# pswpswpsw/nif

Hardware: AMD Instinct MI355X
Metric: train-step points/sec (1D-wave, batch=1M per GPU) (higher is better)
Workload: dtype f32

## Files before the change

nif_amd/csrc/k_pnet_bf16.h:

```cpp
#pragma once
#include "nif_internal.h"

typedef __bf16 pbf16x8 __attribute__((ext_vector_type(8)));
#define PBF_FWD_U4 (3 * 2 * 64)
#define PBF_BWD_U4 (2 * 2 * 64)

__device__ __forceinline__ int pbf_feat(int m, int hf, int t) { return 16 * m + 8 * (t >> 2) + 4 * hf + (t & 3); }

__device__ __forceinline__ void pbf_build(pbf16x8* fwd, pbf16x8* bwd, const float* __restrict__ theta, long w_off, int nst,
                                          int tid, int nthreads) {
  __bf16* f16 = reinterpret_cast<__bf16*>(fwd);
  __bf16* b16 = reinterpret_cast<__bf16*>(bwd);
  for (int e = tid; e < 2 * 64 * 8; e += nthreads) {
    const int t = e & 7, lane = (e >> 3) & 63, m = e >> 9;
    const int row = lane & 31, kf = pbf_feat(m, lane >> 5, t);
    {
      const float w = (kf < nst && row < nst) ? theta[w_off + (long)kf * nst + row] : 0.f;
      const __bf16 w0 = (__bf16)w;
      const float r1 = w - (float)w0;
      const __bf16 w1 = (__bf16)r1;
      f16[((0 * 2 + m) * 64 + lane) * 8 + t] = w0;
      f16[((1 * 2 + m) * 64 + lane) * 8 + t] = w1;
      f16[((2 * 2 + m) * 64 + lane) * 8 + t] = (__bf16)(r1 - (float)w1);
    }
    if (bwd) {
      const float w = (kf < nst && row < nst) ? theta[w_off + (long)row * nst + kf] : 0.f;
      const __bf16 w0 = (__bf16)w;
      b16[((0 * 2 + m) * 64 + lane) * 8 + t] = w0;
      b16[((1 * 2 + m) * 64 + lane) * 8 + t] = (__bf16)(w - (float)w0);
    }
  }
}

__device__ __forceinline__ void pbf_dense_fwd(const pbf16x8* fwd, const f32x16& h, f32x16& T, int lane) {
  pbf16x8 x0[2], x1[2], x2[2];
#pragma unroll
  for (int m = 0; m < 2; ++m)
#pragma unroll
    for (int t = 0; t < 8; ++t) {
      const float x = h[8 * m + t];
      const __bf16 a = (__bf16)x;
      const float r1 = x - (float)a;
      const __bf16 b = (__bf16)r1;
      x0[m][t] = a; x1[m][t] = b; x2[m][t] = (__bf16)(r1 - (float)b);
    }
  f32x16 acc;
#pragma unroll
  for (int e = 0; e < 16; ++e) acc[e] = 0.f;
  const pbf16x8 w0a = fwd[(0 * 2 + 0) * 64 + lane], w0b = fwd[(0 * 2 + 1) * 64 + lane];
  const pbf16x8 w1a = fwd[(1 * 2 + 0) * 64 + lane], w1b = fwd[(1 * 2 + 1) * 64 + lane];
  const pbf16x8 w2a = fwd[(2 * 2 + 0) * 64 + lane], w2b = fwd[(2 * 2 + 1) * 64 + lane];
  acc = __builtin_amdgcn_mfma_f32_32x32x16_bf16(w1a, x1[0], acc, 0, 0, 0);
  acc = __builtin_amdgcn_mfma_f32_32x32x16_bf16(w1b, x1[1], acc, 0, 0, 0);
  acc = __builtin_amdgcn_mfma_f32_32x32x16_bf16(w2a, x0[0], acc, 0, 0, 0);
  acc = __builtin_amdgcn_mfma_f32_32x32x16_bf16(w2b, x0[1], acc, 0, 0, 0);
  acc = __builtin_amdgcn_mfma_f32_32x32x16_bf16(w0a, x2[0], acc, 0, 0, 0);
  acc = __builtin_amdgcn_mfma_f32_32x32x16_bf16(w0b, x2[1], acc, 0, 0, 0);
  acc = __builtin_amdgcn_mfma_f32_32x32x16_bf16(w1a, x0[0], acc, 0, 0, 0);
  acc = __builtin_amdgcn_mfma_f32_32x32x16_bf16(w1b, x0[1], acc, 0, 0, 0);
  acc = __builtin_amdgcn_mfma_f32_32x32x16_bf16(w0a, x1[0], acc, 0, 0, 0);
  acc = __builtin_amdgcn_mfma_f32_32x32x16_bf16(w0b, x1[1], acc, 0, 0, 0);
  acc = __builtin_amdgcn_mfma_f32_32x32x16_bf16(w0a, x0[0], acc, 0, 0, 0);
  acc = __builtin_amdgcn_mfma_f32_32x32x16_bf16(w0b, x0[1], acc, 0, 0, 0);
  T = acc;
}

__device__ __forceinline__ void pbf_dense_bwd(const pbf16x8* bwd, const f32x16& ga, f32x16& U, int lane) {
  pbf16x8 x0[2], x1[2];
#pragma unroll
  for (int m = 0; m < 2; ++m)
#pragma unroll
    for (int t = 0; t < 8; ++t) {
      const float x = ga[8 * m + t];
      const __bf16 a = (__bf16)x;
      x0[m][t] = a; x1[m][t] = (__bf16)(x - (float)a);
    }
  f32x16 acc;
#pragma unroll
  for (int e = 0; e < 16; ++e) acc[e] = 0.f;
  const pbf16x8 w0a = bwd[(0 * 2 + 0) * 64 + lane], w0b = bwd[(0 * 2 + 1) * 64 + lane];
  const pbf16x8 w1a = bwd[(1 * 2 + 0) * 64 + lane], w1b = bwd[(1 * 2 + 1) * 64 + lane];
  acc = __builtin_amdgcn_mfma_f32_32x32x16_bf16(w1a, x0[0], acc, 0, 0, 0);
  acc = __builtin_amdgcn_mfma_f32_32x32x16_bf16(w1b, x0[1], acc, 0, 0, 0);
  acc = __builtin_amdgcn_mfma_f32_32x32x16_bf16(w0a, x1[0], acc, 0, 0, 0);
  acc = __builtin_amdgcn_mfma_f32_32x32x16_bf16(w0b, x1[1], acc, 0, 0, 0);
  acc = __builtin_amdgcn_mfma_f32_32x32x16_bf16(w0a, x0[0], acc, 0, 0, 0);
  acc = __builtin_amdgcn_mfma_f32_32x32x16_bf16(w0b, x0[1], acc, 0, 0, 0);
  U = acc;
}

template <int NB>
__device__ __forceinline__ void pbfn_build_fwd(pbf16x8* fwd, const float* __restrict__ theta, long w_off, int nst, int tid, int nthreads) {
  __bf16* f16 = reinterpret_cast<__bf16*>(fwd);
  for (int e = tid; e < NB * NB * 1024; e += nthreads) {
    const int t = e & 7, lane = (e >> 3) & 63, m = (e >> 9) & 1, blk = e >> 10;
    const int ob = blk / NB, ib = blk - ob * NB;
    const int row = 32 * ob + (lane & 31), kf = 32 * ib + pbf_feat(m, lane >> 5, t);
    const float w = (kf < nst && row < nst) ? theta[w_off + (long)kf * nst + row] : 0.f;
    const __bf16 w0 = (__bf16)w;
    const float r1 = w - (float)w0;
    const __bf16 w1 = (__bf16)r1;
    __bf16* q = f16 + (long)blk * PBF_FWD_U4 * 8;
    q[((0 * 2 + m) * 64 + lane) * 8 + t] = w0;
    q[((1 * 2 + m) * 64 + lane) * 8 + t] = w1;
    q[((2 * 2 + m) * 64 + lane) * 8 + t] = (__bf16)(r1 - (float)w1);
  }
}
template <int NB>
__device__ __forceinline__ void pbfn_dense_fwd(const pbf16x8* fwd, const f32x16 (&h)[NB], f32x16 (&T)[NB], int lane) {
  pbf16x8 x0[NB][2], x1[NB][2], x2[NB][2];
#pragma unroll
  for (int ib = 0; ib < NB; ++ib)
#pragma unroll
    for (int m = 0; m < 2; ++m)
#pragma unroll
      for (int t = 0; t < 8; ++t) {
        const float x = h[ib][8 * m + t];
        const __bf16 a = (__bf16)x;
        const float r1 = x - (float)a;
        const __bf16 b = (__bf16)r1;
        x0[ib][m][t] = a; x1[ib][m][t] = b; x2[ib][m][t] = (__bf16)(r1 - (float)b);
      }
#pragma unroll
  for (int ob = 0; ob < NB; ++ob) {
    f32x16 acc;
#pragma unroll
    for (int e = 0; e < 16; ++e) acc[e] = 0.f;
#pragma unroll
    for (int ib = 0; ib < NB; ++ib) {
      const pbf16x8* q = fwd + (long)(ob * NB + ib) * PBF_FWD_U4;
      const pbf16x8 w0a = q[(0 * 2 + 0) * 64 + lane], w0b = q[(0 * 2 + 1) * 64 + lane];
      const pbf16x8 w1a = q[(1 * 2 + 0) * 64 + lane], w1b = q[(1 * 2 + 1) * 64 + lane];
      const pbf16x8 w2a = q[(2 * 2 + 0) * 64 + lane], w2b = q[(2 * 2 + 1) * 64 + lane];
      acc = __builtin_amdgcn_mfma_f32_32x32x16_bf16(w1a, x1[ib][0], acc, 0, 0, 0);
      acc = __builtin_amdgcn_mfma_f32_32x32x16_bf16(w1b, x1[ib][1], acc, 0, 0, 0);
      acc = __builtin_amdgcn_mfma_f32_32x32x16_bf16(w2a, x0[ib][0], acc, 0, 0, 0);
      acc = __builtin_amdgcn_mfma_f32_32x32x16_bf16(w2b, x0[ib][1], acc, 0, 0, 0);
      acc = __builtin_amdgcn_mfma_f32_32x32x16_bf16(w0a, x2[ib][0], acc, 0, 0, 0);
      acc = __builtin_amdgcn_mfma_f32_32x32x16_bf16(w0b, x2[ib][1], acc, 0, 0, 0);
      acc = __builtin_amdgcn_mfma_f32_32x32x16_bf16(w1a, x0[ib][0], acc, 0, 0, 0);
      acc = __builtin_amdgcn_mfma_f32_32x32x16_bf16(w1b, x0[ib][1], acc, 0, 0, 0);
      acc = __builtin_amdgcn_mfma_f32_32x32x16_bf16(w0a, x1[ib][0], acc, 0, 0, 0);
      acc = __builtin_amdgcn_mfma_f32_32x32x16_bf16(w0b, x1[ib][1], acc, 0, 0, 0);
      acc = __builtin_amdgcn_mfma_f32_32x32x16_bf16(w0a, x0[ib][0], acc, 0, 0, 0);
      acc = __builtin_amdgcn_mfma_f32_32x32x16_bf16(w0b, x0[ib][1], acc, 0, 0, 0);
    }
    T[ob] = acc;
  }
}
```

nif_amd/csrc/k_pnetbw.hip:

```cpp
#include "nif_internal.h"
#include "k_pnet_bf16.h"

struct PbwArgs {
  PNetArgs p;
  float* partial; long pstride;
  const float* touch; long touch_floats;
};

__device__ __forceinline__ f32x4 lds4(const float* q) { return *reinterpret_cast<const f32x4*>(q); }

__device__ __forceinline__ int pswz(int f, int p) { return f * 32 + ((((p >> 2) ^ (f & 7))) << 2) + (p & 3); }
__device__ __forceinline__ int pswz4(int f, int c) { return f * 32 + ((c ^ (f & 7)) << 2); }
__device__ __forceinline__ void tile_store(float* __restrict__ t, const f32x16& h, int p, int hf) {
#pragma unroll
  for (int v = 0; v < 16; ++v) t[pswz(fmap(v, hf), p)] = h[v];
}

typedef __bf16 pbw_bf16x8 __attribute__((ext_vector_type(8)));
__device__ __forceinline__ void grad_mfma(const float* IN, const float* DA, f32x16& C, int i, int hf, int in_rows = 32) {
  f32x4 a[4], b[4];
#pragma unroll
  for (int q = 0; q < 4; ++q) {
    a[q] = lds4(IN + pswz4(i < in_rows ? i : 0, 4 * hf + q));
    if (i >= in_rows) { a[q][0] = 0.f; a[q][1] = 0.f; a[q][2] = 0.f; a[q][3] = 0.f; }
    b[q] = lds4(DA + pswz4(i, 4 * hf + q));
  }
#pragma unroll
  for (int hh = 0; hh < 2; ++hh) {
    pbw_bf16x8 ah, al, bh, bl;
#pragma unroll
    for (int e = 0; e < 8; ++e) {
      const float x = a[2 * hh + (e >> 2)][e & 3], y = b[2 * hh + (e >> 2)][e & 3];
      const __bf16 x0 = (__bf16)x, y0 = (__bf16)y;
      ah[e] = x0; al[e] = (__bf16)(x - (float)x0);
      bh[e] = y0; bl[e] = (__bf16)(y - (float)y0);
    }
    C = __builtin_amdgcn_mfma_f32_32x32x16_bf16(ah, bl, C, 0, 0, 0);
    C = __builtin_amdgcn_mfma_f32_32x32x16_bf16(al, bh, C, 0, 0, 0);
    C = __builtin_amdgcn_mfma_f32_32x32x16_bf16(ah, bh, C, 0, 0, 0);
  }
}
__device__ __forceinline__ float col_sum(const float* DA, int i, int hf) {
  float s = 0.f;
#pragma unroll
  for (int q = 0; q < 4; ++q) { const f32x4 b = lds4(DA + pswz4(i, 4 * hf + q)); s += (b[0] + b[1]) + (b[2] + b[3]); }
  return s;
}

#ifndef NIF_PBW_DZR
#define NIF_PBW_DZR 8
#endif
#ifndef NIF_PBW_WAVES
#define NIF_PBW_WAVES 8
#endif
template <int NM, bool RES, int ACT, bool SMALL>
__global__ __launch_bounds__(64 * NIF_PBW_WAVES) void k_pnet_bwg(PbwArgs G) {
  const PNetArgs& A = G.p;
  extern __shared__ __attribute__((aligned(16))) float lds[];
  constexpr int WV = NIF_PBW_WAVES;
  __shared__ float red[(WV - 1) * 64];
  const int lane = threadIdx.x & 63, wid = threadIdx.x >> 6;
  const int p = lane & 31, hf = lane >> 5, i = p;
  const long ntiles = (A.B + 31) / 32;
  constexpr int WLDS = (NM + 2) * 1024 + 256;
  float* hs = lds + (long)wid * WLDS;
  float* gaT = hs + (NM + 1) * 1024;
  float* xT = gaT + 1024;

  f32x16 C[NM], C1, Cb, CB1;
  float gbh[NM], gb0 = 0.f, gbb = 0.f;
#pragma unroll
  for (int e = 0; e < 16; ++e) { C1[e] = 0.f; Cb[e] = 0.f; CB1[e] = 0.f; }
#pragma unroll
  for (int m = 0; m < NM; ++m) {
    gbh[m] = 0.f;
#pragma unroll
    for (int e = 0; e < 16; ++e) C[m][e] = 0.f;
  }
  for (int q = lane; q < 256; q += 64) xT[q] = 0.f;
  const PSmall S = psmall_stage<1>(A, lds + (long)WV * WLDS, threadIdx.x, 64 * WV);
  f32x4* wpl = reinterpret_cast<f32x4*>(lds + (long)WV * WLDS + ((psmall_floats(A, 1) + 3) & ~3));
  pbf16x8* bpl = reinterpret_cast<pbf16x8*>(wpl);
#pragma unroll
  for (int m = 0; m < NM; ++m) {
    const long w_off = RES ? (m == 0 ? A.hid_w[0] : A.hid_w2[0]) : A.hid_w[m];
    pbf_build(bpl + m * (PBF_FWD_U4 + PBF_BWD_U4), bpl + m * (PBF_FWD_U4 + PBF_BWD_U4) + PBF_FWD_U4, A.theta, w_off, A.nst,
              threadIdx.x, 64 * WV);
  }
  auto dense_f = [&](int m, const f32x16 (&x)[1], f32x16 (&y)[1]) { pbf_dense_fwd(bpl + m * (PBF_FWD_U4 + PBF_BWD_U4), x[0], y[0], lane); };
  auto dense_b = [&](int m, const f32x16 (&x)[1], f32x16 (&y)[1]) { pbf_dense_bwd(bpl + m * (PBF_FWD_U4 + PBF_BWD_U4) + PBF_FWD_U4, x[0], y[0], lane); };
  __syncthreads();

  for (long tile = (long)blockIdx.x * WV + wid; tile < ntiles; tile += (long)gridDim.x * WV) {
    const long pt = tile * 32 + p;
    const long ptc = pt < A.B ? pt : A.B - 1;
    const float* prow = A.xin + ptc * A.ncol + A.col0;
    float dzr[NIF_PBW_DZR];
    if (!SMALL) {
      const float* dzg = A.DZ + tile * A.r * 32;
      const int nd = A.r * 32;
#pragma unroll
      for (int q = 0; q < NIF_PBW_DZR; ++q) { const int e = lane + 64 * q; dzr[q] = e < nd ? dzg[e] : 0.f; }
    }
    f32x16 h[1], T[1], d[NM + 1][1];
    {
      f32x16 acc;
#pragma unroll
      for (int v = 0; v < 16; ++v) acc[v] = 0.f;
      for (int dd = 0; dd < A.pi; ++dd) acc += prow[dd] * psmall_get(S.fw + dd * 32, 0, hf);
      h[0] = A.omega * acc + psmall_get(S.fb, 0, hf);
    }
    act_tile_sel<1, ACT>(A.act, h, h, d[0], A.nst, hf);
    float* park = hs + NM * 1024;
    if (SMALL) {
#pragma unroll
      for (int v = 0; v < 16; ++v) park[v * 64 + lane] = d[0][0][v];
    }
    if (!SMALL && hf == 0) {
      for (int dd = 0; dd < A.pi; ++dd) xT[pswz(dd, p)] = prow[dd];
      xT[pswz(A.pi, p)] = 1.0f;
    }
    if (!RES) {
#pragma unroll
      for (int m = 0; m < NM; ++m) {
        tile_store(hs + m * 1024, h[0], p, hf);
        dense_f(m, h, T);
        T[0] = A.omega * T[0] + psmall_get(S.hb + m * 32, 0, hf);
        act_tile_sel<1, ACT>(A.act, T, T, d[m + 1], A.nst, hf);
        h[0] = A.siren ? T[0] : h[0] + T[0];
      }
    } else {
      f32x16 t[1];
      tile_store(hs, h[0], p, hf);
      dense_f(0, h, T);
      T[0] = A.omega * T[0] + psmall_get(S.hb, 0, hf);
      act_tile_sel<1, ACT>(A.act, T, t, d[1], A.nst, hf);
      tile_store(hs + 1024, t[0], p, hf);
      dense_f(1, t, T);
      {
        const f32x16 lin = A.omega * T[0] + psmall_get(S.hb2, 0, hf);
        T[0] = A.siren ? lin : h[0] + lin;
      }
      act_tile_sel<1, ACT>(A.act, T, T, d[NM], A.nst, hf);
      h[0] = A.siren ? 0.5f * (h[0] + T[0]) : T[0];
    }
    if (!SMALL) tile_store(hs + NM * 1024, h[0], p, hf);
    f32x16 gh[1], ga[1], U[1];
#pragma unroll
    for (int v = 0; v < 16; ++v) gh[0][v] = 0.f;
    if (!SMALL) {
#pragma unroll
      for (int q = 0; q < NIF_PBW_DZR; ++q) gaT[pswz(2 * q + hf, p)] = dzr[q];
#pragma unroll
      for (int q = NIF_PBW_DZR; q < 16; ++q) {
        const int e = lane + 64 * q;
        gaT[pswz(2 * q + hf, p)] = e < A.r * 32 ? A.DZ[tile * A.r * 32 + e] : 0.f;
      }
      for (int c = 0; c < A.r; ++c) gh[0] += gaT[pswz(c, p)] * psmall_get(S.bw + c * 32, 0, hf);
    } else {
      gh[0] += A.DZ[tile * 32 + p] * psmall_get(S.bw, 0, hf);
    }
    if (SMALL) {
      const float dz = A.DZ[tile * 32 + p];
      Cb += dz * h[0];
      gbb += hf == 0 ? dz : 0.f;
    } else {
      grad_mfma(hs + NM * 1024, gaT, Cb, i, hf);
      gbb += col_sum(gaT, i, hf);
    }
    float tv[4] = {0.f, 0.f, 0.f, 0.f};
    if (G.touch) {
      const float* tb = G.touch + tile * G.touch_floats + lane * 16;
#pragma unroll
      for (int q = 0; q < 4; ++q) tv[q] = tb[q * 1024 < G.touch_floats ? q * 1024 : 0];
    }
    if (!RES) {
#pragma unroll
      for (int m = NM - 1; m >= 0; --m) {
        ga[0] = gh[0] * d[m + 1][0];
        tile_store(gaT, ga[0], p, hf);
        grad_mfma(hs + m * 1024, gaT, C[m], i, hf);
        gbh[m] += col_sum(gaT, i, hf);
        dense_b(m, ga, U);
        gh[0] = A.siren ? A.omega * U[0] : gh[0] + A.omega * U[0];
      }
    } else {
      const float half = A.siren ? 0.5f : 1.0f;
      ga[0] = half * gh[0] * d[NM][0];
      tile_store(gaT, ga[0], p, hf);
      grad_mfma(hs + 1024, gaT, C[NM - 1], i, hf);
      gbh[NM - 1] += col_sum(gaT, i, hf);
      dense_b(1, ga, U);
      f32x16 skip;
      skip = A.siren ? 0.5f * gh[0] : ga[0];
      ga[0] = A.omega * U[0] * d[1][0];
      tile_store(gaT, ga[0], p, hf);
      grad_mfma(hs, gaT, C[0], i, hf);
      gbh[0] += col_sum(gaT, i, hf);
      dense_b(0, ga, U);
      gh[0] = skip + A.omega * U[0];
    }
    if (SMALL) {
#pragma unroll
      for (int v = 0; v < 16; ++v) ga[0][v] = gh[0][v] * park[v * 64 + lane];
    } else {
      ga[0] = gh[0] * d[0][0];
    }
    if (SMALL) {
      C1 += prow[0] * ga[0];
      CB1 += ga[0];
    } else {
      tile_store(gaT, ga[0], p, hf);
      grad_mfma(xT, gaT, C1, i, hf, 8);
    }
    asm volatile("" ::"v"(tv[0]), "v"(tv[1]), "v"(tv[2]), "v"(tv[3]));
  }

  float* prow_out = G.partial + (long)blockIdx.x * G.pstride;
  auto sum8 = [&](float v) -> float {
    if (wid > 0) red[(wid - 1) * 64 + lane] = v;
    __syncthreads();
    if (wid == 0) {
#pragma unroll
      for (int w = 0; w < WV - 1; ++w) v += red[w * 64 + lane];
    }
    __syncthreads();
    return v;
  };
  __syncthreads();
  auto sum16 = [&](f32x16 v) -> f32x16 {
    if (wid > 0) {
#pragma unroll
      for (int e = 0; e < 16; ++e) lds[((wid - 1) * 16 + e) * 64 + lane] = v[e];
    }
    __syncthreads();
    if (wid == 0) {
#pragma unroll
      for (int w = 0; w < WV - 1; ++w)
#pragma unroll
        for (int e = 0; e < 16; ++e) v[e] += lds[(w * 16 + e) * 64 + lane];
    }
    __syncthreads();
    return v;
  };
#pragma unroll
  for (int m = 0; m < NM; ++m) {
    const long w_off = RES ? (m == 0 ? A.hid_w[0] : A.hid_w2[0]) : A.hid_w[m];
    const long b_off = RES ? (m == 0 ? A.hid_b[0] : A.hid_b2[0]) : A.hid_b[m];
    {
      const f32x16 vs = sum16(C[m]);
#pragma unroll
      for (int e = 0; e < 16; ++e) {
        const int in = fmap(e, hf), out = i;
        if (wid == 0 && in < A.nst && out < A.nst) prow_out[w_off + (long)in * A.nst + out] = A.omega * vs[e];
      }
    }
    float vb = gbh[m];
    vb += __shfl_xor(vb, 32);
    vb = sum8(vb);
    if (wid == 0 && hf == 0 && i < A.nst) prow_out[b_off + i] = vb;
  }
  if (SMALL) {
    auto lanes32 = [&](f32x16 v) -> f32x16 {
#pragma unroll
      for (int off = 16; off > 0; off >>= 1)
#pragma unroll
        for (int e = 0; e < 16; ++e) v[e] += __shfl_xor(v[e], off);
      return v;
    };
    const f32x16 s1 = sum16(lanes32(C1)), s0 = sum16(lanes32(CB1)), sb = sum16(lanes32(Cb));
#pragma unroll
    for (int e = 0; e < 16; ++e) {
      const int f = fmap(e, hf);
      if (wid == 0 && p == 0 && f < A.nst) {
        prow_out[A.first_w + f] = A.omega * s1[e];
        prow_out[A.first_b + f] = s0[e];
        prow_out[A.bott_w + f] = sb[e];
      }
    }
    float v = gbb;
#pragma unroll
    for (int off = 32; off > 0; off >>= 1) v += __shfl_xor(v, off);
    v = sum8(v);
    if (wid == 0 && lane == 0) prow_out[A.bott_b] = v;
    return;
  }
  const f32x16 s1 = sum16(C1), sb = sum16(Cb);
#pragma unroll
  for (int e = 0; e < 16; ++e) {
    const float v1 = s1[e];
    const float vb = sb[e];
    const int row = fmap(e, hf);
    if (wid == 0) {
      if (row < A.pi && i < A.nst) prow_out[A.first_w + (long)row * A.nst + i] = A.omega * v1;
      if (row == A.pi && i < A.nst) prow_out[A.first_b + i] = v1;
      if (row < A.nst && i < A.r) prow_out[A.bott_w + (long)row * A.r + i] = vb;
    }
  }
  (void)gb0;
  {
    float v = gbb;
    v += __shfl_xor(v, 32);
    v = sum8(v);
    if (wid == 0 && hf == 0 && i < A.r) prow_out[A.bott_b + i] = v;
  }
}

bool pnet_bwg_supported(const PNetArgs& a) {
  const int nm = a.lst * (a.res ? 2 : 1);
  return a.nst <= 32 && a.pi <= 6 && a.r <= 32 && nm >= 1 && nm <= 2 && (!a.res || a.lst == 1);
}

void launch_pnet_bwg(const PNetArgs& a, float* partial, long pstride, int rows, hipStream_t st, const float* touch,
                     long touch_floats) {
  PbwArgs G; G.p = a; G.partial = partial; G.pstride = pstride; G.touch = touch; G.touch_floats = touch_floats;
  const int nm = a.lst * (a.res ? 2 : 1);
  dim3 grid(rows), block(64 * NIF_PBW_WAVES);
  const size_t shm = ((size_t)NIF_PBW_WAVES * ((nm + 2) * 1024 + 256) + (size_t)((psmall_floats(a, 1) + 3) & ~3) +
                      (size_t)nm * 2560) * sizeof(float);
#define PBW1(NM_, RES_, ACT_, SM_)                                                                                  \
  {                                                                                                                 \
    (void)hipFuncSetAttribute((const void*)k_pnet_bwg<NM_, RES_, ACT_, SM_>, hipFuncAttributeMaxDynamicSharedMemorySize, (int)shm); \
    hipLaunchKernelGGL((k_pnet_bwg<NM_, RES_, ACT_, SM_>), grid, block, shm, st, G);                                \
  }
#define PBW(NM_, RES_, ACT_)                                                                                        \
  {                                                                                                                 \
    if (a.pi == 1 && a.r == 1) PBW1(NM_, RES_, ACT_, true) else PBW1(NM_, RES_, ACT_, false)                        \
  }
#define PBWA(NM_, RES_)                                                       \
  if (a.act == ACT_SWISH) PBW(NM_, RES_, ACT_SWISH)                           \
  else if (a.act == ACT_SINE) PBW(NM_, RES_, ACT_SINE)                        \
  else PBW(NM_, RES_, -1)
  if (a.res) { PBWA(2, true) }
  else if (nm == 1) { PBWA(1, false) }
  else { PBWA(2, false) }
#undef PBWA
#undef PBW
#undef PBW1
}
```

Baseline: 942.3 million.

## Exchange bf16-split activations via LDS transpose reads for weight-gradient MFMAs

```diff
diff --git a/nif_amd/csrc/k_pnet_bf16.h b/nif_amd/csrc/k_pnet_bf16.h
--- a/nif_amd/csrc/k_pnet_bf16.h
+++ b/nif_amd/csrc/k_pnet_bf16.h
@@ -32,8 +32,7 @@
   }
 }
 
-__device__ __forceinline__ void pbf_dense_fwd(const pbf16x8* fwd, const f32x16& h, f32x16& T, int lane) {
-  pbf16x8 x0[2], x1[2], x2[2];
+__device__ __forceinline__ void pbf_split3(const f32x16& h, pbf16x8 (&x0)[2], pbf16x8 (&x1)[2], pbf16x8 (&x2)[2]) {
 #pragma unroll
   for (int m = 0; m < 2; ++m)
 #pragma unroll
@@ -44,6 +43,20 @@
       const __bf16 b = (__bf16)r1;
       x0[m][t] = a; x1[m][t] = b; x2[m][t] = (__bf16)(r1 - (float)b);
     }
+}
+__device__ __forceinline__ void pbf_split2(const f32x16& h, pbf16x8 (&x0)[2], pbf16x8 (&x1)[2]) {
+#pragma unroll
+  for (int m = 0; m < 2; ++m)
+#pragma unroll
+    for (int t = 0; t < 8; ++t) {
+      const float x = h[8 * m + t];
+      const __bf16 a = (__bf16)x;
+      x0[m][t] = a; x1[m][t] = (__bf16)(x - (float)a);
+    }
+}
+
+__device__ __forceinline__ void pbf_dense_fwd(const pbf16x8* fwd, const pbf16x8 (&x0)[2], const pbf16x8 (&x1)[2],
+                                              const pbf16x8 (&x2)[2], f32x16& T, int lane) {
   f32x16 acc;
 #pragma unroll
   for (int e = 0; e < 16; ++e) acc[e] = 0.f;
@@ -64,17 +77,13 @@
   acc = __builtin_amdgcn_mfma_f32_32x32x16_bf16(w0b, x0[1], acc, 0, 0, 0);
   T = acc;
 }
+__device__ __forceinline__ void pbf_dense_fwd(const pbf16x8* fwd, const f32x16& h, f32x16& T, int lane) {
+  pbf16x8 x0[2], x1[2], x2[2];
+  pbf_split3(h, x0, x1, x2);
+  pbf_dense_fwd(fwd, x0, x1, x2, T, lane);
+}
 
-__device__ __forceinline__ void pbf_dense_bwd(const pbf16x8* bwd, const f32x16& ga, f32x16& U, int lane) {
-  pbf16x8 x0[2], x1[2];
-#pragma unroll
-  for (int m = 0; m < 2; ++m)
-#pragma unroll
-    for (int t = 0; t < 8; ++t) {
-      const float x = ga[8 * m + t];
-      const __bf16 a = (__bf16)x;
-      x0[m][t] = a; x1[m][t] = (__bf16)(x - (float)a);
-    }
+__device__ __forceinline__ void pbf_dense_bwd(const pbf16x8* bwd, const pbf16x8 (&x0)[2], const pbf16x8 (&x1)[2], f32x16& U, int lane) {
   f32x16 acc;
 #pragma unroll
   for (int e = 0; e < 16; ++e) acc[e] = 0.f;
@@ -87,6 +96,11 @@
   acc = __builtin_amdgcn_mfma_f32_32x32x16_bf16(w0a, x0[0], acc, 0, 0, 0);
   acc = __builtin_amdgcn_mfma_f32_32x32x16_bf16(w0b, x0[1], acc, 0, 0, 0);
   U = acc;
+}
+__device__ __forceinline__ void pbf_dense_bwd(const pbf16x8* bwd, const f32x16& ga, f32x16& U, int lane) {
+  pbf16x8 x0[2], x1[2];
+  pbf_split2(ga, x0, x1);
+  pbf_dense_bwd(bwd, x0, x1, U, lane);
 }
 
 template <int NB>
diff --git a/nif_amd/csrc/k_pnet_xchg.h b/nif_amd/csrc/k_pnet_xchg.h
--- /dev/null
+++ b/nif_amd/csrc/k_pnet_xchg.h
@@ -0,0 +1,55 @@
+#pragma once
+
+#if !defined(__HIPCC__) && !defined(__host__)
+#define __host__
+#define __device__
+#endif
+
+#define PXC_QUAD_STRIDE 544
+#define PXC_PLANE_BYTES 2176
+
+__host__ __device__ inline int pxc_unit(int p, int g, int hf) {
+  return PXC_QUAD_STRIDE * g + 256 * (p >> 4) + 128 * hf + 32 * ((p >> 2) & 3) + 8 * (p & 3);
+}
+__host__ __device__ inline int pxc_dep_addr(int lane) { return pxc_unit(lane & 31, 0, lane >> 5); }
+__host__ __device__ inline int pxc_rd_addr(int lane) {
+  const int grp = lane >> 4, s = lane & 15;
+  const int quad = 4 * (grp & 1) + (s & 3);
+  return pxc_unit(16 * (grp >> 1) + (s >> 2), quad >> 1, quad & 1);
+}
+#define PXC_RD_STEP 64
+#define PXC_RD_HALF 32
+
+#ifdef __HIPCC__
+typedef __bf16 pxc_bf16x8 __attribute__((ext_vector_type(8)));
+typedef __bf16 pxc_bf16x4 __attribute__((ext_vector_type(4)));
+typedef __bf16 pxc_bf16x2 __attribute__((ext_vector_type(2)));
+
+__device__ __forceinline__ void pxc_deposit(char* img, int dep, const pxc_bf16x8 (&s)[2]) {
+  typedef unsigned long long u64;
+#pragma unroll
+  for (int m = 0; m < 2; ++m) {
+    const u64 lo = __builtin_bit_cast(u64, __builtin_shufflevector(s[m], s[m], 0, 1, 2, 3));
+    const u64 hi = __builtin_bit_cast(u64, __builtin_shufflevector(s[m], s[m], 4, 5, 6, 7));
+    *reinterpret_cast<u64*>(img + dep + PXC_QUAD_STRIDE * (2 * m)) = lo;
+    *reinterpret_cast<u64*>(img + dep + PXC_QUAD_STRIDE * (2 * m + 1)) = hi;
+  }
+}
+__device__ __forceinline__ pxc_bf16x8 pxc_read_op(const char* img, int rd, int s) {
+  typedef __attribute__((address_space(3))) pxc_bf16x4* lds_p;
+  const pxc_bf16x4 x0 = __builtin_amdgcn_ds_read_tr16_b64_v4bf16((lds_p)(img + rd + PXC_RD_STEP * s));
+  const pxc_bf16x4 x1 = __builtin_amdgcn_ds_read_tr16_b64_v4bf16((lds_p)(img + rd + PXC_RD_STEP * s + PXC_RD_HALF));
+  return __builtin_shufflevector(x0, x1, 0, 1, 2, 3, 4, 5, 6, 7);
+}
+__device__ __forceinline__ float pxc_sum8(const pxc_bf16x8 hi, const pxc_bf16x8 lo, float acc) {
+  const __bf16 one = (__bf16)1.0f;
+  const pxc_bf16x2 ones = {one, one};
+#pragma unroll
+  for (int e = 0; e < 8; e += 2) {
+    const pxc_bf16x2 a = {hi[e], hi[e + 1]}, b = {lo[e], lo[e + 1]};
+    acc = __builtin_amdgcn_fdot2_f32_bf16(a, ones, acc, false);
+    acc = __builtin_amdgcn_fdot2_f32_bf16(b, ones, acc, false);
+  }
+  return acc;
+}
+#endif
diff --git a/nif_amd/csrc/k_pnetbw.hip b/nif_amd/csrc/k_pnetbw.hip
--- a/nif_amd/csrc/k_pnetbw.hip
+++ b/nif_amd/csrc/k_pnetbw.hip
@@ -1,5 +1,6 @@
 #include "nif_internal.h"
 #include "k_pnet_bf16.h"
+#include "k_pnet_xchg.h"
 
 struct PbwArgs {
   PNetArgs p;
@@ -11,41 +12,39 @@
 
 __device__ __forceinline__ int pswz(int f, int p) { return f * 32 + ((((p >> 2) ^ (f & 7))) << 2) + (p & 3); }
 __device__ __forceinline__ int pswz4(int f, int c) { return f * 32 + ((c ^ (f & 7)) << 2); }
-__device__ __forceinline__ void tile_store(float* __restrict__ t, const f32x16& h, int p, int hf) {
-#pragma unroll
-  for (int v = 0; v < 16; ++v) t[pswz(fmap(v, hf), p)] = h[v];
-}
-
-typedef __bf16 pbw_bf16x8 __attribute__((ext_vector_type(8)));
-__device__ __forceinline__ void grad_mfma(const float* IN, const float* DA, f32x16& C, int i, int hf, int in_rows = 32) {
-  f32x4 a[4], b[4];
-#pragma unroll
-  for (int q = 0; q < 4; ++q) {
-    a[q] = lds4(IN + pswz4(i < in_rows ? i : 0, 4 * hf + q));
-    if (i >= in_rows) { a[q][0] = 0.f; a[q][1] = 0.f; a[q][2] = 0.f; a[q][3] = 0.f; }
-    b[q] = lds4(DA + pswz4(i, 4 * hf + q));
-  }
-#pragma unroll
-  for (int hh = 0; hh < 2; ++hh) {
-    pbw_bf16x8 ah, al, bh, bl;
-#pragma unroll
-    for (int e = 0; e < 8; ++e) {
-      const float x = a[2 * hh + (e >> 2)][e & 3], y = b[2 * hh + (e >> 2)][e & 3];
-      const __bf16 x0 = (__bf16)x, y0 = (__bf16)y;
-      ah[e] = x0; al[e] = (__bf16)(x - (float)x0);
-      bh[e] = y0; bl[e] = (__bf16)(y - (float)y0);
-    }
-    C = __builtin_amdgcn_mfma_f32_32x32x16_bf16(ah, bl, C, 0, 0, 0);
-    C = __builtin_amdgcn_mfma_f32_32x32x16_bf16(al, bh, C, 0, 0, 0);
-    C = __builtin_amdgcn_mfma_f32_32x32x16_bf16(ah, bh, C, 0, 0, 0);
-  }
-}
-__device__ __forceinline__ float col_sum(const float* DA, int i, int hf) {
-  float s = 0.f;
-#pragma unroll
-  for (int q = 0; q < 4; ++q) { const f32x4 b = lds4(DA + pswz4(i, 4 * hf + q)); s += (b[0] + b[1]) + (b[2] + b[3]); }
-  return s;
-}
+
+struct GOp { pbf16x8 hi[2], lo[2]; };
+__device__ __forceinline__ GOp gop_xchg(const char* img, int rd) {
+  GOp o;
+#pragma unroll
+  for (int s = 0; s < 2; ++s) { o.hi[s] = pxc_read_op(img, rd, s); o.lo[s] = pxc_read_op(img + PXC_PLANE_BYTES, rd, s); }
+  return o;
+}
+__device__ __forceinline__ GOp gop_f32(const float* T, int i, int hf, int rows = 32) {
+  GOp o;
+#pragma unroll
+  for (int s = 0; s < 2; ++s)
+#pragma unroll
+    for (int q = 0; q < 2; ++q) {
+      f32x4 a = lds4(T + pswz4(i < rows ? i : 0, 4 * hf + 2 * s + q));
+      if (i >= rows) { a[0] = 0.f; a[1] = 0.f; a[2] = 0.f; a[3] = 0.f; }
+#pragma unroll
+      for (int e = 0; e < 4; ++e) {
+        const __bf16 x0 = (__bf16)a[e];
+        o.hi[s][4 * q + e] = x0; o.lo[s][4 * q + e] = (__bf16)(a[e] - (float)x0);
+      }
+    }
+  return o;
+}
+__device__ __forceinline__ void grad_mfma(const GOp& in, const GOp& da, f32x16& C) {
+#pragma unroll
+  for (int s = 0; s < 2; ++s) {
+    C = __builtin_amdgcn_mfma_f32_32x32x16_bf16(in.hi[s], da.lo[s], C, 0, 0, 0);
+    C = __builtin_amdgcn_mfma_f32_32x32x16_bf16(in.lo[s], da.hi[s], C, 0, 0, 0);
+    C = __builtin_amdgcn_mfma_f32_32x32x16_bf16(in.hi[s], da.hi[s], C, 0, 0, 0);
+  }
+}
+__device__ __forceinline__ float col_sum(const GOp& da) { return pxc_sum8(da.hi[1], da.lo[1], pxc_sum8(da.hi[0], da.lo[0], 0.f)); }
 
 #ifndef NIF_PBW_DZR
 #define NIF_PBW_DZR 8
@@ -53,6 +52,8 @@
 #ifndef NIF_PBW_WAVES
 #define NIF_PBW_WAVES 8
 #endif
+__host__ __device__ constexpr int pbw_wave_floats(int nm) { return (2 * nm + 2) * (PXC_PLANE_BYTES / 4) + 1024; }
+
 template <int NM, bool RES, int ACT, bool SMALL>
 __global__ __launch_bounds__(64 * NIF_PBW_WAVES) void k_pnet_bwg(PbwArgs G) {
   const PNetArgs& A = G.p;
@@ -62,13 +63,14 @@
   const int lane = threadIdx.x & 63, wid = threadIdx.x >> 6;
   const int p = lane & 31, hf = lane >> 5, i = p;
   const long ntiles = (A.B + 31) / 32;
-  constexpr int WLDS = (NM + 2) * 1024 + 256;
-  float* hs = lds + (long)wid * WLDS;
-  float* gaT = hs + (NM + 1) * 1024;
-  float* xT = gaT + 1024;
+  constexpr int WLDS = pbw_wave_floats(NM);
+  char* xh = reinterpret_cast<char*>(lds + (long)wid * WLDS);
+  char* xa = xh + 2 * NM * PXC_PLANE_BYTES;
+  float* gaT = reinterpret_cast<float*>(xa + 2 * PXC_PLANE_BYTES);
+  const int dep = pxc_dep_addr(lane), rd = pxc_rd_addr(lane);
 
   f32x16 C[NM], C1, Cb, CB1;
-  float gbh[NM], gb0 = 0.f, gbb = 0.f;
+  float gbh[NM], gbb = 0.f;
 #pragma unroll
   for (int e = 0; e < 16; ++e) { C1[e] = 0.f; Cb[e] = 0.f; CB1[e] = 0.f; }
 #pragma unroll
@@ -77,7 +79,6 @@
 #pragma unroll
     for (int e = 0; e < 16; ++e) C[m][e] = 0.f;
   }
-  for (int q = lane; q < 256; q += 64) xT[q] = 0.f;
   const PSmall S = psmall_stage<1>(A, lds + (long)WV * WLDS, threadIdx.x, 64 * WV);
   f32x4* wpl = reinterpret_cast<f32x4*>(lds + (long)WV * WLDS + ((psmall_floats(A, 1) + 3) & ~3));
   pbf16x8* bpl = reinterpret_cast<pbf16x8*>(wpl);
@@ -87,8 +88,30 @@
     pbf_build(bpl + m * (PBF_FWD_U4 + PBF_BWD_U4), bpl + m * (PBF_FWD_U4 + PBF_BWD_U4) + PBF_FWD_U4, A.theta, w_off, A.nst,
               threadIdx.x, 64 * WV);
   }
-  auto dense_f = [&](int m, const f32x16 (&x)[1], f32x16 (&y)[1]) { pbf_dense_fwd(bpl + m * (PBF_FWD_U4 + PBF_BWD_U4), x[0], y[0], lane); };
-  auto dense_b = [&](int m, const f32x16 (&x)[1], f32x16 (&y)[1]) { pbf_dense_bwd(bpl + m * (PBF_FWD_U4 + PBF_BWD_U4) + PBF_FWD_U4, x[0], y[0], lane); };
+  auto dense_f = [&](int m, const f32x16& x, f32x16& y) {
+    pbf16x8 x0[2], x1[2], x2[2];
+    pbf_split3(x, x0, x1, x2);
+    pxc_deposit(xh + 2 * m * PXC_PLANE_BYTES, dep, x0);
+    pxc_deposit(xh + (2 * m + 1) * PXC_PLANE_BYTES, dep, x1);
+    pbf_dense_fwd(bpl + m * (PBF_FWD_U4 + PBF_BWD_U4), x0, x1, x2, y, lane);
+  };
+  auto adjoint = [&](int m, const f32x16& ga, f32x16& U) {
+    pbf16x8 g0[2], g1[2];
+    pbf_split2(ga, g0, g1);
+    pxc_deposit(xa, dep, g0);
+    pxc_deposit(xa + PXC_PLANE_BYTES, dep, g1);
+    const GOp da = gop_xchg(xa, rd);
+    grad_mfma(gop_xchg(xh + 2 * m * PXC_PLANE_BYTES, rd), da, C[m]);
+    gbh[m] += col_sum(da);
+    pbf_dense_bwd(bpl + m * (PBF_FWD_U4 + PBF_BWD_U4) + PBF_FWD_U4, g0, g1, U, lane);
+  };
+  auto xchg_once = [&](const f32x16& t) -> GOp {
+    pbf16x8 t0[2], t1[2];
+    pbf_split2(t, t0, t1);
+    pxc_deposit(xa, dep, t0);
+    pxc_deposit(xa + PXC_PLANE_BYTES, dep, t1);
+    return gop_xchg(xa, rd);
+  };
   __syncthreads();
 
   for (long tile = (long)blockIdx.x * WV + wid; tile < ntiles; tile += (long)gridDim.x * WV) {
@@ -111,32 +134,25 @@
       h[0] = A.omega * acc + psmall_get(S.fb, 0, hf);
     }
     act_tile_sel<1, ACT>(A.act, h, h, d[0], A.nst, hf);
-    float* park = hs + NM * 1024;
+    float* park = gaT;
     if (SMALL) {
 #pragma unroll
       for (int v = 0; v < 16; ++v) park[v * 64 + lane] = d[0][0][v];
     }
-    if (!SMALL && hf == 0) {
-      for (int dd = 0; dd < A.pi; ++dd) xT[pswz(dd, p)] = prow[dd];
-      xT[pswz(A.pi, p)] = 1.0f;
-    }
     if (!RES) {
 #pragma unroll
       for (int m = 0; m < NM; ++m) {
-        tile_store(hs + m * 1024, h[0], p, hf);
-        dense_f(m, h, T);
+        dense_f(m, h[0], T[0]);
         T[0] = A.omega * T[0] + psmall_get(S.hb + m * 32, 0, hf);
         act_tile_sel<1, ACT>(A.act, T, T, d[m + 1], A.nst, hf);
         h[0] = A.siren ? T[0] : h[0] + T[0];
       }
     } else {
       f32x16 t[1];
-      tile_store(hs, h[0], p, hf);
-      dense_f(0, h, T);
+      dense_f(0, h[0], T[0]);
       T[0] = A.omega * T[0] + psmall_get(S.hb, 0, hf);
       act_tile_sel<1, ACT>(A.act, T, t, d[1], A.nst, hf);
-      tile_store(hs + 1024, t[0], p, hf);
-      dense_f(1, t, T);
+      dense_f(1, t[0], T[0]);
       {
         const f32x16 lin = A.omega * T[0] + psmall_get(S.hb2, 0, hf);
         T[0] = A.siren ? lin : h[0] + lin;
@@ -144,7 +160,6 @@
       act_tile_sel<1, ACT>(A.act, T, T, d[NM], A.nst, hf);
       h[0] = A.siren ? 0.5f * (h[0] + T[0]) : T[0];
     }
-    if (!SMALL) tile_store(hs + NM * 1024, h[0], p, hf);
     f32x16 gh[1], ga[1], U[1];
 #pragma unroll
     for (int v = 0; v < 16; ++v) gh[0][v] = 0.f;
@@ -165,8 +180,9 @@
       Cb += dz * h[0];
       gbb += hf == 0 ? dz : 0.f;
     } else {
-      grad_mfma(hs + NM * 1024, gaT, Cb, i, hf);
-      gbb += col_sum(gaT, i, hf);
+      const GOp dz = gop_f32(gaT, i, hf);
+      grad_mfma(xchg_once(h[0]), dz, Cb);
+      gbb += col_sum(dz);
     }
     float tv[4] = {0.f, 0.f, 0.f, 0.f};
     if (G.touch) {
@@ -178,40 +194,32 @@
 #pragma unroll
       for (int m = NM - 1; m >= 0; --m) {
         ga[0] = gh[0] * d[m + 1][0];
-        tile_store(gaT, ga[0], p, hf);
-        grad_mfma(hs + m * 1024, gaT, C[m], i, hf);
-        gbh[m] += col_sum(gaT, i, hf);
-        dense_b(m, ga, U);
+        adjoint(m, ga[0], U[0]);
         gh[0] = A.siren ? A.omega * U[0] : gh[0] + A.omega * U[0];
       }
     } else {
       const float half = A.siren ? 0.5f : 1.0f;
       ga[0] = half * gh[0] * d[NM][0];
-      tile_store(gaT, ga[0], p, hf);
-      grad_mfma(hs + 1024, gaT, C[NM - 1], i, hf);
-      gbh[NM - 1] += col_sum(gaT, i, hf);
-      dense_b(1, ga, U);
+      adjoint(1, ga[0], U[0]);
       f32x16 skip;
       skip = A.siren ? 0.5f * gh[0] : ga[0];
       ga[0] = A.omega * U[0] * d[1][0];
-      tile_store(gaT, ga[0], p, hf);
-      grad_mfma(hs, gaT, C[0], i, hf);
-      gbh[0] += col_sum(gaT, i, hf);
-      dense_b(0, ga, U);
+      adjoint(0, ga[0], U[0]);
       gh[0] = skip + A.omega * U[0];
     }
     if (SMALL) {
 #pragma unroll
       for (int v = 0; v < 16; ++v) ga[0][v] = gh[0][v] * park[v * 64 + lane];
-    } else {
-      ga[0] = gh[0] * d[0][0];
-    }
-    if (SMALL) {
       C1 += prow[0] * ga[0];
       CB1 += ga[0];
     } else {
-      tile_store(gaT, ga[0], p, hf);
-      grad_mfma(xT, gaT, C1, i, hf, 8);
+      ga[0] = gh[0] * d[0][0];
+#pragma unroll
+      for (int q = 0; q < 4; ++q) {
+        const int row = 4 * hf + q;
+        gaT[pswz(row, p)] = row < A.pi ? prow[row] : (row == A.pi ? 1.0f : 0.f);
+      }
+      grad_mfma(gop_f32(gaT, i, hf, 8), xchg_once(ga[0]), C1);
     }
     asm volatile("" ::"v"(tv[0]), "v"(tv[1]), "v"(tv[2]), "v"(tv[3]));
   }
@@ -297,7 +305,6 @@
       if (row < A.nst && i < A.r) prow_out[A.bott_w + (long)row * A.r + i] = vb;
     }
   }
-  (void)gb0;
   {
     float v = gbb;
     v += __shfl_xor(v, 32);
@@ -316,7 +323,7 @@
   PbwArgs G; G.p = a; G.partial = partial; G.pstride = pstride; G.touch = touch; G.touch_floats = touch_floats;
   const int nm = a.lst * (a.res ? 2 : 1);
   dim3 grid(rows), block(64 * NIF_PBW_WAVES);
-  const size_t shm = ((size_t)NIF_PBW_WAVES * ((nm + 2) * 1024 + 256) + (size_t)((psmall_floats(a, 1) + 3) & ~3) +
+  const size_t shm = ((size_t)NIF_PBW_WAVES * pbw_wave_floats(nm) + (size_t)((psmall_floats(a, 1) + 3) & ~3) +
                       (size_t)nm * 2560) * sizeof(float);
 #define PBW1(NM_, RES_, ACT_, SM_)                                                                                  \
   {                                                                                                                 \
```

Result: no change. 947.7 million (median of 6 runs) (+0.6%).
